# Icelk/fractal-renderer

Measured on AMD Instinct MI355X. Metric: pixel_iterations_per_sec, higher is better.
Workload: dtype f64

## Files before the change

fractal-renderer_amd/csrc/fr_api.hip:

```cpp
#include <hip/hip_runtime.h>

#include <atomic>
#include <cmath>
#include <cstddef>
#include <cstdint>
#include <cstdio>
#include <cstdlib>
#include <cstring>
#include <mutex>
#include <shared_mutex>
#include <string>
#include <vector>

#include "fr_ctx.h"

static_assert(sizeof(fr_config) == 104 && offsetof(fr_config, limit) == 16 && offsetof(fr_config, inside) == 72 &&
                  offsetof(fr_config, primary_color) == 74 && offsetof(fr_config, color_weight) == 80 &&
                  offsetof(fr_config, julia_set) == 88,
              "fr_config must stay the #[repr(C)] image of calc::Config");
static_assert(sizeof(fr_render_opts) == 32, "fr_render_opts is part of the ABI");

namespace fr {

namespace {

thread_local std::string tl_error;
thread_local Profiling tl_prof;
std::atomic<bool> g_process_exiting{false};

std::shared_mutex g_life;
std::mutex g_primary_mu;
Ctx g_primary;
bool g_primary_inited = false;

std::atomic<int> g_tile{0};
std::atomic<int> g_palette_enabled{1};
std::atomic<int> g_cycle_shortcut{0};
std::atomic<int> g_refill_minrun{-1}, g_refill_quit16{-1};
std::atomic<int> g_loop_mode{-1};
std::atomic<int> g_colour_filter{1};
std::atomic<unsigned long long *> g_queue_trace{nullptr};
std::atomic<uint32_t> g_two_pass_list_entries{0};

bool valid_tile(int tile) {
    switch (tile) {
    case 0: case 1: case 2: case 4: case 8: case 9: case 10: case 11: case 12: case 13: case 14: case 15: case 16: case 6401: case 3202: case 1604: case 808:
        return true;
    default:
        return false;
    }
}

}

int fail(int code, const char *what) {
    tl_error = what;
    return code;
}
int fail(int code, const std::string &what) {
    tl_error = what;
    return code;
}

int fail_hip(hipError_t e, const char *what) {
    char buf[512];
    snprintf(buf, sizeof buf, "%s: %s (%s)", what, hipGetErrorString(e), hipGetErrorName(e));
    tl_error = buf;
    (void)hipGetLastError();
    return (e == hipErrorNoDevice || e == hipErrorInvalidDevice) ? FR_ERR_NO_DEVICE : FR_ERR_HIP;
}

const std::string &last_error() { return tl_error; }

LifeShared::LifeShared() { g_life.lock_shared(); }
LifeShared::~LifeShared() { g_life.unlock_shared(); }
LifeExclusive::LifeExclusive() { g_life.lock(); }
LifeExclusive::~LifeExclusive() { g_life.unlock(); }

Profiling &profiling() { return tl_prof; }
Profiling::~Profiling() {
    if (e0 && !g_process_exiting.load()) {
        (void)hipEventDestroy(e0);
        (void)hipEventDestroy(e1);
    }
    e0 = e1 = nullptr;
}

Opts default_opts() {
    Opts o;
    o.tile = g_tile.load();
    o.loop_mode = g_loop_mode.load();
    o.palette = g_palette_enabled.load();
    o.cycle_shortcut = g_cycle_shortcut.load();
    o.refill_minrun = g_refill_minrun.load();
    o.refill_quit16 = g_refill_quit16.load();
    o.colour_filter = g_colour_filter.load();
    return o;
}

int resolve_opts(const fr_render_opts *in, Opts &o) {
    o = default_opts();
    if (!in) return FR_OK;
    if (in->size < sizeof(fr_render_opts)) return fail(FR_ERR_INVALID_ARGUMENT, "fr_render_opts.size is too small (use fr_render_opts_init)");
    if (!valid_tile(in->tile)) return fail(FR_ERR_INVALID_ARGUMENT, "opts.tile must be 0, 1, 2, 4, 8, 9, 10 ... 16, 6401, 3202, 1604 or 808");
    if (in->loop_mode != -1 && in->loop_mode != 0 && in->loop_mode != 2 && in->loop_mode != 4 && in->loop_mode != 5)
        return fail(FR_ERR_INVALID_ARGUMENT, "opts.loop_mode must be -1 (auto), 0, 2, 4 or 5");
    if (in->refill_minrun < -1 || in->refill_quit16 < -1 || in->refill_quit16 == 0 || in->refill_quit16 > 16)
        return fail(FR_ERR_INVALID_ARGUMENT, "opts: refill_minrun >= 0, 1 <= refill_quit16 <= 16 (or -1: the kernel's default)");
    o.tile = in->tile;
    o.loop_mode = in->loop_mode;
    o.palette = in->palette != 0;
    o.cycle_shortcut = in->cycle_shortcut != 0;
    o.refill_minrun = in->refill_minrun;
    o.refill_quit16 = in->refill_quit16;
    o.colour_filter = in->colour_filter == 2 ? 2 : in->colour_filter != 0;
    return FR_OK;
}


int Ctx::create(int device) {
    HIP_TRY(hipSetDevice(device));
    hip_device = device;
    HIP_TRY(hipStreamCreateWithFlags(&stream, hipStreamNonBlocking));
    HIP_TRY(hipStreamCreateWithFlags(&stream2, hipStreamNonBlocking));
    int prio_least = 0, prio_greatest = 0;
    if (hipDeviceGetStreamPriorityRange(&prio_least, &prio_greatest) != hipSuccess) {
        (void)hipGetLastError();
        prio_greatest = 0;
    }
    HIP_TRY(hipStreamCreateWithPriority(&copy_stream, hipStreamNonBlocking, prio_greatest));
    HIP_TRY(hipStreamCreateWithPriority(&aux_stream, hipStreamNonBlocking, prio_greatest));
    HIP_TRY(hipStreamCreateWithPriority(&aux2_stream, hipStreamNonBlocking, prio_least));
    HIP_TRY(hipMalloc(reinterpret_cast<void **>(&sample_counters), 16 * sizeof(unsigned long long)));
    HIP_TRY(hipMemset(sample_counters, 0, 16 * sizeof(unsigned long long)));
    HIP_TRY(hipHostMalloc(reinterpret_cast<void **>(&sample_result), (kViewChoices + 1) * 8 * sizeof(unsigned long long), hipHostMallocMapped));
    memset(sample_result, 0, (kViewChoices + 1) * 8 * sizeof(unsigned long long));
    for (ViewChoice &v : view_choices) HIP_TRY(hipEventCreateWithFlags(&v.after, hipEventDisableTiming));
    constexpr size_t kSlotWords = FR_MAX_PALETTE_ENTRIES + FR_SURV_QUEUES * FR_SURV_COUNT_STRIDE;
    HIP_TRY(hipMalloc(reinterpret_cast<void **>(&palette_block), sizeof(uint32_t) * kSlotWords * kPaletteSlots));
    for (int k = 0; k < kPaletteSlots; k++) {
        palette_slots[k].dev = palette_block + (size_t)k * kSlotWords;
        HIP_TRY(hipEventCreateWithFlags(&palette_slots[k].done, hipEventDisableTiming));
// ... 319 lines not shown
    p.pos_re = cfg->pos.re;
    p.pos_im = cfg->pos.im;
    p.scale_re = cfg->scale.re;
    p.scale_im = cfg->scale.im;
    p.exposure = cfg->exposure;
    p.julia_re = cfg->julia_set.re;
    p.julia_im = cfg->julia_set.im;
    p.inside = cfg->inside ? 1u : 0u;
    p.smooth = cfg->smooth ? 1u : 0u;
    p.prim[0] = cfg->primary_color.r;
    p.prim[1] = cfg->primary_color.g;
    p.prim[2] = cfg->primary_color.b;
    p.sec[0] = cfg->secondary_color.r;
    p.sec[1] = cfg->secondary_color.g;
    p.sec[2] = cfg->secondary_color.b;
    for (int k = 0; k < 3; k++) {
        p.prim_f[k] = (double)p.prim[k];
        p.sec_f[k] = (double)p.sec[k];
    }
    p.iterations_f64 = (double)cfg->iterations;
    const uint32_t n = cfg->iterations;
    p.inv_iterations = (n != 0 && (n & (n - 1)) == 0) ? 1.0 / (double)n : 0.0;
    p.ncols = cfg->width;
    p.nrows = 0;
    p.x_first = 0;
    p.x_stride = 1;
    p.block_rows = 1;
    p.y_first = 0;
    p.y_stride = 1;
    p.refill_minrun = o.refill_minrun < 0 ? 32u : (uint32_t)o.refill_minrun;
    p.refill_quit16 = o.refill_quit16 < 0 ? 8u : (uint32_t)o.refill_quit16;
    p.queue_minrun = (o.refill_minrun < 0 || (o.tile >= 11 && o.tile <= 16)) ? 8u : (uint32_t)o.refill_minrun;
    p.first_keep = ((o.tile >= 11 && o.tile <= 16) && o.refill_quit16 > 0) ? 4u * (uint32_t)o.refill_quit16 : 0u;
    p.two_pass_cap = ((o.tile >= 11 && o.tile <= 16) && o.refill_minrun > 0) ? (uint32_t)o.refill_minrun : 0u;
    p.queue_want = (o.refill_quit16 < 0 || (o.tile >= 11 && o.tile <= 16)) ? 24u : (64u * (uint32_t)o.refill_quit16 + 15u) / 16u;
    {
        static const int dbg_want = getenv("FR_DEBUG_QUEUE_WANT") ? atoi(getenv("FR_DEBUG_QUEUE_WANT")) : 0;
        static const int dbg_minrun = getenv("FR_DEBUG_QUEUE_MINRUN") ? atoi(getenv("FR_DEBUG_QUEUE_MINRUN")) : -1;
        if (dbg_want > 0 && dbg_want <= 64) p.queue_want = (uint32_t)dbg_want;
        if (dbg_minrun >= 0) p.queue_minrun = (uint32_t)dbg_minrun;
    }
    {
        static const int dbg_ablate = getenv("FR_DEBUG_ABLATE") ? atoi(getenv("FR_DEBUG_ABLATE")) : 0;
        p.debug_ablate = (uint32_t)dbg_ablate & 3u;
    }
    p.cycle_shortcut = (o.cycle_shortcut && cfg->iterations < (1u << 30)) ? 1u : 0u;
    p.filt_k = n != 0 ? cfg->exposure / (double)n : 0.0;
    const bool filter_ok = o.colour_filter && cfg->smooth && n != 0 && std::isfinite(cfg->exposure) &&
                           std::fabs(p.filt_k) <= 1e100 && cfg->stable_limit >= 0.0;
    p.colour_filter = filter_ok ? 1u : 0u;
    const double ak = std::fabs(p.filt_k);
    p.colour_filter32 = (filter_ok && o.colour_filter == 1 && n < (1u << 24) && ak >= 0x1p-60 && ak <= 0x1p60) ? 1u : 0u;
    p.filt_k32 = (float)p.filt_k;
    p.filt_c32 = p.colour_filter32 ? std::nextafterf((float)(ak * FR_NU_BRACKET * (1.0 + 0x1p-9)), INFINITY) : 0.0f;
    for (int k = 0; k < 3; k++) {
        p.filt_d[k] = p.prim_f[k] * ak * FR_NU_BRACKET * (1.0 + 0x1p-20);
        p.filt_d32[k] = p.colour_filter32 ? std::nextafterf((float)(p.prim_f[k] * ak * FR_NU_BRACKET * (1.0 + 0x1p-10)), INFINITY) : 0.0f;
        p.prim32[k] = (float)p.prim[k];
    }
    const double lo = std::fmax(cfg->stable_limit, 2.0) * (1.0 + 0x1p-20);
    p.filt_lo32 = (p.colour_filter32 && lo < 1e30) ? std::nextafterf((float)lo, INFINITY) : INFINITY;
}

static double host_coord(double coord, double max, double offset, double pos, double scale) {
    return ((coord / max) - offset) / scale + pos;
}

constexpr uint32_t kSpecQuiet = 16;

void plan_loop(const fr_config *cfg, int precision, const Opts &o, fr_kparams &p) {
    p.loop_mode = 0;
    p.skip_t = 0.0;
    p.loop_spec = 0;
    const bool no_spec = o.loop_mode == 5;
    const int forced = no_spec ? -1 : o.loop_mode;
    if (cfg->algo != FR_ALGO_MANDELBROT && cfg->algo != FR_ALGO_JULIA) return;
    if (p.ncols == 0 || p.nrows == 0) return;
    const bool f32 = precision == FR_PRECISION_F32;
    const double range_hi = f32 ? 0x1p30 : 0x1p400;
    const double slack = f32 ? 1.0 + 0x1p-18 : 1.0 + 0x1p-30;
    double lim2;
    if (f32) {
        const float lf = (float)cfg->limit;
        lim2 = (double)(lf * lf);
    } else {
        lim2 = cfg->limit * cfg->limit;
    }
    auto mag = [f32](double v) { return std::fabs(f32 ? (double)(float)v : v); };
    const double w = (double)cfg->width, h = (double)cfg->height;
    const uint64_t x_last = (uint64_t)p.x_first + (uint64_t)(p.ncols - 1) * p.x_stride;
    const uint32_t r_last = p.nrows - 1;
    const uint64_t y_last = (uint64_t)p.y_first + (uint64_t)(r_last / p.block_rows) * p.y_stride + r_last % p.block_rows;
    if (x_last > 0xFFFFFFFFull || y_last > 0xFFFFFFFFull) return;
    auto nmax = [](double a, double b) { return (a != a || b != b) ? NAN : std::fmax(a, b); };
    double smax = 0.0;
    for (double x : {(double)p.x_first, (double)x_last})
        smax = nmax(smax, mag(host_coord(x, h, (w / h) / 2.0, cfg->pos.re, cfg->scale.re)));
    for (double y : {(double)p.y_first, (double)y_last})
        smax = nmax(smax, mag(host_coord(y, h, 0.5, cfg->pos.im, cfg->scale.im)));
    const double cmax = cfg->algo == FR_ALGO_JULIA ? nmax(mag(cfg->julia_set.re), mag(cfg->julia_set.im)) : smax;
    if (!no_spec && lim2 >= 16.0 && lim2 <= (f32 ? 0x1p100 : 0x1p1000) && cmax <= lim2 / 8.0 && smax <= (f32 ? 0x1p120 : 0x1p1000)) {
        static const int dbg = getenv("FR_DEBUG_SPEC_QUIET") ? atoi(getenv("FR_DEBUG_SPEC_QUIET")) : 0;
        p.loop_spec = dbg > 0 ? (uint32_t)dbg : kSpecQuiet;
    }
    if (forced == 0) return;
    if (!(std::fabs(cfg->limit) <= range_hi)) return;
    if (!(cmax <= range_hi)) return;
    for (int m : {4, 2}) {
        if (forced > 0 && forced != m) continue;
        double d = lim2;
        for (int j = 1; j < m && d > 0.0; j++) d = std::sqrt(d / (2.0 * slack)) - cmax;
        double t = d * (1.0 - 0x1p-20);
        if (f32) {
            float tf = (float)t;
            if ((double)tf > t) tf = std::nextafterf(tf, 0.0f);
            t = (double)tf;
        }
        if (t >= 4.5 || (forced == m && t > 0.0)) {
            p.loop_mode = (uint32_t)m;
            p.skip_t = t;
            if (!(t < lim2)) p.loop_spec = 0;
            return;
        }
    }
}

static int check_rows(const fr_config *cfg, uint32_t y0, uint32_t y1) {
    if (!cfg) return fail(FR_ERR_INVALID_ARGUMENT, "cfg is NULL");
    if (y0 > y1) return fail(FR_ERR_INVALID_ARGUMENT, "y0 > y1");
    if (y1 > cfg->height) return fail(FR_ERR_INVALID_ARGUMENT, "y1 > height");
    return FR_OK;
}

int check_precision(int precision) {
    if (precision == FR_PRECISION_DD)
        return fail(FR_ERR_INVALID_ARGUMENT, "FR_PRECISION_DD is single-device only: the row renders, fr_pixel_p, fr_escape_rows(_dd) "
                                             "and fr_count_iterations take it");
    if (precision == FR_PRECISION_PT)
        return fail(FR_ERR_INVALID_ARGUMENT, "FR_PRECISION_PT is single-device only: the row renders, fr_pixel_p, fr_escape_rows(_pt) "
                                             "and fr_count_iterations take it");
    if (precision != FR_PRECISION_F64 && precision != FR_PRECISION_F32)
        return fail(FR_ERR_INVALID_ARGUMENT, "precision must be FR_PRECISION_F64 or FR_PRECISION_F32");
    return FR_OK;
}

static int check_deep(const fr_config *cfg, const fr_imaginary *pos_lo, const char *name) {
    if (!cfg) return fail(FR_ERR_INVALID_ARGUMENT, "cfg is NULL");
    const std::string n(name);
    const double lo_re = pos_lo ? pos_lo->re : 0.0, lo_im = pos_lo ? pos_lo->im : 0.0;
    const double fields[] = {cfg->limit,    cfg->stable_limit, cfg->pos.re,       cfg->pos.im,       cfg->scale.re, cfg->scale.im,
                             cfg->exposure, cfg->color_weight, cfg->julia_set.re, cfg->julia_set.im, lo_re,         lo_im};
    for (double v : fields)
        if (!std::isfinite(v)) return fail(FR_ERR_INVALID_ARGUMENT, n + ": every field of the view must be finite");
    if (!(cfg->limit > 0.0 && cfg->limit <= 0x1p500))
// ... 446 lines not shown
    snprintf(buf, buf_len, "%s", prop.gcnArchName);
    return FR_OK;
}

void fr_config_new(fr_config *cfg, uint32_t algo) {
    if (!cfg) return;
    const bool fern = algo == FR_ALGO_BARNSLEY_FERN;
    memset(cfg, 0, sizeof *cfg);
    cfg->algo = algo;
    cfg->width = 2000;
    cfg->height = 1000;
    cfg->iterations = fern ? 10000000u : 50u;
    cfg->limit = 65536.0;
    cfg->stable_limit = 2.0;
    cfg->scale.re = 0.4;
    cfg->scale.im = 0.4;
    cfg->exposure = 2.0;
    cfg->inside = 1;
    cfg->smooth = 1;
    if (fern) {
        cfg->primary_color = fr_rgb{4, 3, 100};
        cfg->secondary_color = fr_rgb{240, 240, 240};
    } else {
        cfg->primary_color = fr_rgb{40, 255, 40};
        cfg->secondary_color = fr_rgb{240, 0, 170};
    }
    cfg->color_weight = 0.01;
}

void fr_render_opts_init(fr_render_opts *opts) {
    if (!opts) return;
    const Opts o = default_opts();
    opts->size = sizeof(fr_render_opts);
    opts->tile = o.tile;
    opts->loop_mode = o.loop_mode;
    opts->palette = o.palette;
    opts->cycle_shortcut = o.cycle_shortcut;
    opts->refill_minrun = o.refill_minrun;
    opts->refill_quit16 = o.refill_quit16;
    opts->colour_filter = o.colour_filter;
}


static int render_rows_device(const fr_config *cfg, int precision, uint32_t y0, uint32_t y1, void *d_out,
                              size_t out_len, void *hip_stream, unsigned bytes_per_pixel, const fr_render_opts *opts,
                              const fr_imaginary *pos_lo = nullptr) {
    int rc = check_rows(cfg, y0, y1);
    if (rc == FR_OK) rc = check_precision_lo(cfg, precision, pos_lo);
    Opts o;
    if (rc == FR_OK) rc = resolve_opts(opts, o);
    if (rc != FR_OK) return rc;
    const size_t need = (size_t)bytes_per_pixel * cfg->width * (size_t)(y1 - y0);
    if (need == 0) return FR_OK;
    if (!d_out) return fail(FR_ERR_INVALID_ARGUMENT, "d_out is NULL");
    if (out_len < need) return fail(FR_ERR_BUFFER_TOO_SMALL, "out_len < bytes_per_pixel*width*(y1-y0)");
    if (bytes_per_pixel == 4 && (reinterpret_cast<uintptr_t>(d_out) & 3u))
        return fail(FR_ERR_INVALID_ARGUMENT, "RGBA8 output must be 4-byte aligned");
    LifeShared ls;
    Ctx *ctx;
    rc = primary(&ctx);
    if (rc != FR_OK) return rc;
    if (precision == FR_PRECISION_DD || precision == FR_PRECISION_PT)
        return render_deep_device(*ctx, precision, cfg, pos_lo, o, y0, y1, bytes_per_pixel, d_out,
                                  static_cast<hipStream_t>(hip_stream));
    fr_kparams p;
    fill_params(cfg, o, p);
    p.nrows = y1 - y0;
// ... 371 lines not shown

int fr_set_profiling(int enabled) {
    Profiling &pr = profiling();
    pr.enabled = enabled != 0;
    if (!enabled) {
        pr.have = false;
        if (pr.e0) {
            (void)hipEventDestroy(pr.e0);
            (void)hipEventDestroy(pr.e1);
            pr.e0 = pr.e1 = nullptr;
        }
    }
    return FR_OK;
}

int fr_last_kernel_ms(float *ms) {
    if (!ms) return fail(FR_ERR_INVALID_ARGUMENT, "ms is NULL");
    Profiling &pr = profiling();
    if (!pr.have) return fail(FR_ERR_INVALID_ARGUMENT, "no profiled kernel on this thread");
    HIP_TRY(hipEventSynchronize(pr.e1));
    HIP_TRY(hipEventElapsedTime(ms, pr.e0, pr.e1));
    return FR_OK;
}

int fr_last_kernel_name(char *buf, size_t buf_len) {
    if (!buf || buf_len == 0) return fail(FR_ERR_INVALID_ARGUMENT, "buf is NULL or empty");
    Profiling &pr = profiling();
    if (!pr.have) return fail(FR_ERR_INVALID_ARGUMENT, "no profiled kernel on this thread");
    snprintf(buf, buf_len, "%s", pr.kernel);
    return FR_OK;
}

int fr_set_tile(int tile) {
    if (!valid_tile(tile)) return fail(FR_ERR_INVALID_ARGUMENT, "tile must be 0, 1, 2, 4, 8, 9, 10 ... 16, 6401, 3202, 1604 or 808");
    g_tile.store(tile);
    return FR_OK;
}

int fr_set_refill_policy(int minrun, int quit16) {
    if (minrun < -1 || quit16 < -1 || quit16 == 0 || quit16 > 16)
        return fail(FR_ERR_INVALID_ARGUMENT, "minrun >= 0, 1 <= quit16 <= 16 (or -1: the kernel's default)");
    g_refill_minrun.store(minrun);
    g_refill_quit16.store(quit16);
    return FR_OK;
}

int fr_set_cycle_shortcut(int enabled) {
    g_cycle_shortcut.store(enabled ? 1 : 0);
    return FR_OK;
}

int fr_set_palette(int enabled) {
    g_palette_enabled.store(enabled ? 1 : 0);
    return FR_OK;
}

int fr_set_colour_filter(int enabled) {
    g_colour_filter.store(enabled == 2 ? 2 : enabled ? 1 : 0);
    return FR_OK;
}

int fr_set_loop_mode(int mode) {
    if (mode != -1 && mode != 0 && mode != 2 && mode != 4 && mode != 5)
        return fail(FR_ERR_INVALID_ARGUMENT, "loop mode must be -1 (auto), 0, 2, 4 or 5");
    g_loop_mode.store(mode);
    return FR_OK;
}
// ... 123 lines not shown
```

fractal-renderer_amd/csrc/fr_ctx.h:

```cpp
#ifndef FR_CTX_H
#define FR_CTX_H

#include <hip/hip_runtime.h>

#include <atomic>
#include <cstddef>
#include <cstdint>
#include <memory>
#include <condition_variable>
#include <mutex>
#include <string>
#include <thread>
#include <vector>

#include "../../include/fractal_hip.h"
#include "fr_kernels.h"

namespace fr {

int fail(int code, const char *what);
int fail(int code, const std::string &what);
int fail_hip(hipError_t e, const char *what);
const std::string &last_error();

#define HIP_TRY(expr)                                          \
    do {                                                       \
        hipError_t e_ = (expr);                                \
        if (e_ != hipSuccess) return ::fr::fail_hip(e_, #expr); \
    } while (0)

struct Opts {
    int tile = 0;
    int loop_mode = -1;
    int palette = 1;
    int cycle_shortcut = 0;
    int refill_minrun = -1, refill_quit16 = -1;
    int colour_filter = 1;
    int kernel_hint = -2;
    bool one_band = false;
    bool no_spec = false;
    uint32_t strip_tiles = 0;
    int pending_sample = -1;
};
Opts default_opts();
int resolve_opts(const fr_render_opts *o, Opts &out);

struct Scratch {
    void *ptr = nullptr;
    size_t cap = 0;
};

struct PaletteSlot {
    uint32_t *dev = nullptr;
    hipEvent_t done = nullptr;
    bool pending = false;
    bool busy = false;
};
constexpr int kPaletteSlots = 16;

struct SurvSlot {
    void *dev = nullptr;
    hipEvent_t done = nullptr;
    bool pending = false, busy = false;
};
constexpr int kSurvSlots = 3;
// ... 147 lines not shown
```

fractal-renderer_amd/csrc/fr_kernels.h:

```cpp
#ifndef FR_KERNELS_H
#define FR_KERNELS_H

#include <hip/hip_runtime.h>
#include <stdint.h>

struct fr_kparams {
    uint32_t algo;
    uint32_t width, height;
    uint32_t iterations;
    double limit, stable_limit;
    double pos_re, pos_im, scale_re, scale_im;
    double exposure;
    double julia_re, julia_im;
    uint32_t inside, smooth;
    uint32_t prim[3], sec[3];
    double prim_f[3], sec_f[3];
    double iterations_f64, inv_iterations;
    uint32_t ncols, nrows;
    uint32_t x_first, x_stride;
    uint32_t block_rows, y_first, y_stride;
    uint32_t out_in_place;
    uint32_t out_rgba;
    uint32_t loop_mode;
    double skip_t;
    uint32_t loop_spec;
    uint32_t first_no_spec;
    const uint32_t *palette;
    uint32_t palette_entries;
    uint32_t refill_minrun, refill_quit16;
    uint32_t queue_minrun, queue_want;
    uint32_t cycle_shortcut;
    uint32_t colour_filter;
    uint32_t *work_counter;
    double filt_k;
    double filt_d[3];
    uint32_t colour_filter32;
    float filt_k32;
    float filt_c32;
    float filt_d32[3];
    float prim32[3];
    float filt_lo32;
    uint32_t first_cap;
    uint32_t first_keep;
    uint32_t two_pass_cap;
    uint32_t first_only;
    uint32_t second_v1;
    uint32_t first_one_band;
    uint32_t strip_tiles;
    uint32_t debug_ablate;
    uint32_t surv_sub_capacity;
    void *surv_z;
    uint32_t *surv_pos;
    uint32_t *surv_cnt;
    void *surv_c;
    uint32_t *surv_counts;
};

constexpr uint32_t FR_SURV_QUEUES = 64;
constexpr uint32_t FR_SURV_COUNT_STRIDE = 32;
constexpr uint32_t FR_SURV_CHUNK = 64;

constexpr double FR_NU_BRACKET = 0x1p-18;

enum fr_out_mode {
    FR_OUT_RGB = 0,
    FR_OUT_ESCAPE = 1,
    FR_OUT_COUNT = 2
};

constexpr uint32_t FR_COUNT_SLOTS = 512;

struct fr_kout {
    uint8_t *rgb;
    double *z;
    uint32_t *iters;
    unsigned long long *count;
    unsigned long long *trace;
};

hipError_t fr_launch_escape(const fr_kparams &p, int precision, int mode, const fr_kout &out, int tile,
                            hipStream_t stream, const char **kernel_name);

hipError_t fr_launch_escape_dd(const fr_kparams &p, double pos_lo_re, double pos_lo_im, int mode, const fr_kout &out,
                               bool with_lo, hipStream_t stream, const char **kernel_name);

bool fr_wants_work_queue(const fr_kparams &p, int tile);

bool fr_wants_two_pass(fr_kparams &p, int precision, int tile, int hint = -1);
// ... 31 lines not shown
```

fractal-renderer_amd/csrc/fr_kernels.hip:

```cpp
#include "fr_kernels.h"

#include <cmath>

#include <cstdlib>

#include "fr_math.h"

namespace {

#include "fr_colour.h"

constexpr int kWaves = 4;


#define FR_ORBIT_STEP(SFX, TAG)                    \
    "v_add_" SFX " %[t], %[r2], -%[i2]\n"          \
    "v_add_" SFX " %[x], %[re], %[re]\n"           \
    "v_add_" SFX " %[re], %[t], %[cre]\n"          \
    "v_mul_" SFX " %[x], %[x], %[im]\n"            \
    "v_add_" SFX " %[im], %[x], %[cim]\n"          \
    "v_mul_" SFX " %[r2], %[re], %[re]\n"          \
    "v_mul_" SFX " %[i2], %[im], %[im]\n"          \
    "v_add_" SFX " %[t], %[r2], %[i2]\n"           \
    "s_mov_b64 %[sprev], exec\n"                   \
// ... 559 lines not shown
        const bool ok = valid && d32 >= f.lo && d32 <= 0x1.ffffep119f && decided;
        packed = ok ? pk : 0u;
        todo &= ~ballot64(ok);
    }
    if (todo != 0ull) {
        bool inside_done = false;
        if (lane_in(todo)) {
            double dist;
            if constexpr (sizeof(T) == 8) {
                dist = (double)(r2 + i2);
            } else {
                const double zre = (double)re, zim = (double)im;
                dist = zre * zre + zim * zim;
            }
            FR_COLD_PARAMS(kp);
            inside_done = !(dist > kp->stable_limit);
            if (inside_done && kp->inside)
                packed = sat_u8_dev(kp->sec_f[0] * dist) | (sat_u8_dev(kp->sec_f[2] * dist) << 8) | (sat_u8_dev(kp->sec_f[1] * dist) << 16);
        }
        todo &= ~ballot64(inside_done);
    }
    if (todo != 0ull) {
        if (lane_in(todo)) {
            FR_COLD_PARAMS(kp);
            const ColourConsts cc = make_colour_consts(*kp);
            uint8_t rgb[3];
            colour_pixel<T>(cc, re, im, r2, i2, iters, lds_tab, palette, rgb);
            packed = (uint32_t)rgb[0] | ((uint32_t)rgb[1] << 8) | ((uint32_t)rgb[2] << 16);
        }
    }
    return packed;
}

template <typename T, int MODE>
__device__ __forceinline__ void render_pixel(const fr_kparams &p, const fr_kout &out, const double *s_tab,
                                             const uint32_t *s_pal, double sre, double sim, bool valid,
                                             uint32_t cx, uint32_t r, uint32_t lane, uint32_t r_out,
                                             int strip_scalable = -1, const TileOut *to = nullptr) {
    double zre = 0.0, zim = 0.0;
    T tre = 0, tim = 0, tr2 = 0, ti2 = 0;
    uint32_t iters = 0;
    const bool escape_algo = p.algo == 0  || p.algo == 2 ;
    if (valid && escape_algo) {
        const double cre = p.algo == 0 ? sre : p.julia_re;
        const double cim = p.algo == 0 ? sim : p.julia_im;
        if constexpr (sizeof(T) == 8) {
            tre = sre;
            tim = sim;
            iters = orbit_auto<double>(p.loop_mode, p.iterations, tre, tim, cre, cim, p.limit * p.limit, p.skip_t,
                                       tr2, ti2, strip_scalable, p.loop_spec);
            zre = tre;
            zim = tim;
        } else {
            tre = (float)sre, tim = (float)sim;
            const float lim = (float)p.limit;
            iters = orbit_auto<float>(p.loop_mode, p.iterations, tre, tim, (float)cre, (float)cim, lim * lim,
                                      (float)p.skip_t, tr2, ti2, strip_scalable, p.loop_spec);
            zre = (double)tre;
            zim = (double)tim;
        }
    }

    if constexpr (MODE == FR_OUT_RGB) {
        if (to != nullptr) {
            uint32_t packed = 0;
            if (escape_algo) packed = colour_packed<T>(valid, to->fast_colour, tre, tim, tr2, ti2, iters, s_tab, s_pal);
            if (valid) {
                if (to->narrow) {
                    store_packed(to->base, to->lane_off, packed, to->bpp);
                } else {
                    const uint8_t rgb[3] = {(uint8_t)packed, (uint8_t)(packed >> 8), (uint8_t)(packed >> 16)};
                    store_pixel(p, out.rgb, r_out, cx, rgb);
                }
            }
        } else if (valid) {
            uint8_t rgb[3] = {0, 0, 0};
            if (escape_algo) {
                const ColourConsts cc = make_colour_consts(p);
                colour_pixel<T>(cc, tre, tim, tr2, ti2, iters, s_tab, s_pal, rgb);
            }
            store_pixel(p, out.rgb, r_out, cx, rgb);
        }
    } else if constexpr (MODE == FR_OUT_ESCAPE) {
        if (valid) {
            const uint64_t k = (uint64_t)r * p.ncols + cx;
            if (out.z) {
                out.z[2 * k] = zre;
                out.z[2 * k + 1] = zim;
            }
            if (out.iters) out.iters[k] = iters;
        }
    } else {
        unsigned long long n = 0;
        if (valid && escape_algo) n = iters < p.iterations ? (unsigned long long)iters + 1ull : p.iterations;
        for (int off = 32; off > 0; off >>= 1) n += __shfl_down(n, off, 64);
        if (lane == 0 && n) atomicAdd(out.count + ((blockIdx.x + 131u * blockIdx.y) % FR_COUNT_SLOTS), n);
    }
}

template <typename T, int TW, int TH, int WX, int WY, int MODE>
__global__ __launch_bounds__(64 * kWaves) void escape_kernel(const fr_kparams p, const fr_kout out) {
    static_assert(TW * TH == 64 && WX * WY == kWaves, "one lane per pixel, 4 waves per workgroup");
    constexpr int BW = TW * WX, BH = TH * WY;
    __shared__ double s_tab[FR_LOG2_N * 3];
    __shared__ double s_re[BW];
    __shared__ double s_im[BH];

    const uint32_t tid = threadIdx.x;
    const uint32_t tiles_x = (p.ncols + BW - 1) / BW;
    const uint32_t bx = blockIdx.x % tiles_x, by = blockIdx.x / tiles_x;
    const uint32_t col0 = bx * BW, row0 = by * BH;

    if (MODE == FR_OUT_RGB) {
        const double *gt = &g_log2_tab[0][0];
        for (uint32_t k = tid; k < FR_LOG2_N * 3; k += 64 * kWaves) s_tab[k] = gt[k];
    }
    if (tid < BW + BH) {
        const double width = (double)p.width, height = (double)p.height;
        if (tid < BW) {
            const uint32_t x = p.x_first + (col0 + tid) * p.x_stride;
            s_re[tid] = coord_to_space((double)x, height, (width / height) / 2.0, p.pos_re, p.scale_re);
        } else {
            const uint32_t r = row0 + (tid - BW);
            const uint32_t y = p.y_first + (r / p.block_rows) * p.y_stride + r % p.block_rows;
            s_im[tid - BW] = coord_to_space((double)y, height, 0.5, p.pos_im, p.scale_im);
        }
    }
    __syncthreads();

    const uint32_t wave = tid >> 6, lane = tid & 63;
// ... 2 lines not shown
    const uint32_t cx = col0 + lx, r = row0 + ly;
    const bool valid = cx < p.ncols && r < p.nrows;
    render_pixel<T, MODE>(p, out, s_tab, nullptr, s_re[lx], s_im[ly], valid, cx, r, lane, r);
}

template <typename T>
__device__ __forceinline__ bool coords_admissible(bool julia, double julia_re, double julia_im, double coord, bool relevant) {
    constexpr T lo = ScalableRange<T>::lo, hi = ScalableRange<T>::hi;
    const T v = (T)coord;
    const T av = __builtin_fabs(v);
    const bool in_range = av >= lo && av <= hi;
    bool lane_ok;
    if (julia) {
        const T jr = __builtin_fabs((T)julia_re), ji = __builtin_fabs((T)julia_im);
        lane_ok = (v == (T)0 || in_range) && jr >= lo && jr <= hi && ji >= lo && ji <= hi;
    } else {
        lane_ok = in_range;
    }
    return __ballot(relevant && !lane_ok) == 0ull;
}
template <typename T>
__device__ __forceinline__ bool coords_admissible(const fr_kparams &p, double coord, bool relevant) {
    return coords_admissible<T>(p.algo == 2, p.julia_re, p.julia_im, coord, relevant);
}

template <typename T>
__device__ __forceinline__ bool strip_is_scalable(const fr_kparams &p, double coord_lane, uint32_t tile0, uint32_t row0,
                                                  uint32_t lane) {
    const bool relevant = lane >= 56 ? (row0 + (lane - 56) < p.nrows) : (tile0 * 8u + lane < p.ncols);
    return coords_admissible<T>(p, coord_lane, relevant);
}


template <typename T, int MODE, int kStripTiles>
__global__ __launch_bounds__(64) void escape_strip_kernel(const fr_kparams p, const fr_kout out) {
    __shared__ double s_tab[(FR_LOG2_N * 3 * 8 > FR_MAX_PALETTE_ENTRIES * 4 ? FR_LOG2_N * 3 * 8 : FR_MAX_PALETTE_ENTRIES * 4) / 8];
    const uint32_t tid = threadIdx.x;
    const uint32_t *s_pal = nullptr;
    if (MODE == FR_OUT_RGB) {
        if (p.palette != nullptr) {
            uint32_t *dst = reinterpret_cast<uint32_t *>(s_tab);
            for (uint32_t k = tid; k < p.palette_entries; k += 64) dst[k] = p.palette[k];
            s_pal = dst;
        } else if (p.smooth) {
            const double *gt = &g_log2_tab[0][0];
            for (uint32_t k = tid; k < FR_LOG2_N * 3; k += 64) s_tab[k] = gt[k];
        }
        __syncthreads();
    }
    const uint32_t lane = tid;
    const uint32_t row0 = (blockIdx.y + gridDim.y * blockIdx.z) * 8u;
    if (row0 >= p.nrows) return;
    const uint32_t lx = lane & 7u, ly = lane >> 3;
    const uint32_t r = row0 + ly;
    const double width = (double)p.width, height = (double)p.height;

    static_assert(kStripTiles <= 7, "lanes 56-63 are the row lanes");
    const bool row_lane = lane >= 56;
    const uint32_t tile0 = blockIdx.x * kStripTiles;
    uint32_t coord_u;
    if (row_lane) {
        const uint32_t rr = row0 + (lane - 56);
        coord_u = p.y_first + (rr / p.block_rows) * p.y_stride + rr % p.block_rows;
    } else {
        coord_u = p.x_first + (tile0 * 8u + lane) * p.x_stride;
    }
    const double coord_lane = coord_to_space((double)coord_u, height, row_lane ? 0.5 : (width / height) / 2.0,
                                             row_lane ? p.pos_im : p.pos_re, row_lane ? p.scale_im : p.scale_re);
    const double sim = __shfl(coord_lane, 56 + ly, 64);
    uint32_t out_row0 = row0;
    if (p.out_in_place) out_row0 = p.y_first + (row0 / p.block_rows) * p.y_stride + row0 % p.block_rows;
    const uint32_t r_out = out_row0 + ly;
    const int strip_scalable = (p.loop_mode != 0 && strip_is_scalable<T>(p, coord_lane, tile0, row0, lane)) ? 1 : 0;
    TileOut to;
    to.bpp = p.out_rgba ? 4u : 3u;
    to.narrow = (uint64_t)p.ncols * to.bpp * 8u <= 0xFFFFFFFFull;
    to.lane_off = ly * (p.ncols * to.bpp) + lx * to.bpp;
    to.fast_colour = p.colour_filter32 && p.smooth && p.palette == nullptr;
    uint8_t *const strip_base = MODE == FR_OUT_RGB ? out.rgb + ((uint64_t)out_row0 * p.ncols + (uint64_t)tile0 * 8u) * to.bpp : nullptr;

    for (int k = 0; k < kStripTiles; k++) {
        const uint32_t col0 = (tile0 + k) * 8u;
        if (col0 >= p.ncols) break;
        const double sre = __shfl(coord_lane, k * 8 + lx, 64);
        const uint32_t cx = col0 + lx;
        const bool valid = cx < p.ncols && r < p.nrows;
        to.base = strip_base + (size_t)((uint32_t)k * 8u * to.bpp);
        render_pixel<T, MODE>(p, out, s_tab, s_pal, sre, sim, valid, cx, r, lane, r_out, strip_scalable, MODE == FR_OUT_RGB ? &to : nullptr);
    }
}

__device__ __forceinline__ uint32_t wave_max_u32(uint32_t v) {
    for (int off = 32; off > 0; off >>= 1) {
        const uint32_t o = __shfl_xor(v, off, 64);
        v = o > v ? o : v;
    }
    return v;
}

template <typename T>
struct Pair;
template <>
struct Pair<float> {
    typedef float2 type;
};
template <>
struct Pair<double> {
    typedef double2 type;
};

template <typename T>
__device__ __forceinline__ bool coord_is_scalable(bool julia, double coord) {
    constexpr T lo = ScalableRange<T>::lo, hi = ScalableRange<T>::hi;
    const T v = (T)coord;
    const T av = __builtin_fabs(v);
    const bool in_range = av >= lo && av <= hi;
    return julia ? (v == (T)0 || in_range) : in_range;
}

template <typename T, int M, int kStripTiles, int kBands>
__global__ __launch_bounds__(64) void escape_first_v1_kernel(const fr_kparams p, const fr_kout out) {
// ... 493 lines not shown
#define FR_TILE_OPERANDS                                                                                         \
    : [X] "=&v"(X), [Y] "=&v"(Y), [A] "=&v"(A), [B] "=&v"(B), [t] "=&v"(t), [cnt] "=&v"(cnt), [q] "=&v"(q),      \
      [sorig] "=&s"(sorig), [srun] "=&s"(srun), [k] "+s"(k), [st] "=&s"(st), [fa] "=&s"(fa), [fb] "=&s"(fb),     \
      [fk] "=&s"(fk)                                                                                             \
    : [sre] "v"(sre), [Y0] "v"(Y0), [B0] "v"(B0), [c2re] "v"(c2re), [c2im] "v"(c2im), [t4lim] "s"(t4lim),        \
      [lim4] "s"(lim4), [kargs] "s"(kargs), [offa] "i"(offsetof(fr_kparams, prim32)),                            \
      [offb] "i"(offsetof(fr_kparams, prim32) + 8),                                                              \
      [offk] "i"(offsetof(fr_kparams, filt_k32))                                                                 \
    : "vcc", "scc", "memory"
    if constexpr (sizeof(T) == 8) {
        if constexpr (M == 4)
            asm volatile(FR_TILE_ASM("f64", "v_mov_b64", FR_SC_IT("f64") FR_SC_IT("f64") FR_SC_IT("f64"), "4.0") FR_TILE_OPERANDS);
        else
            asm volatile(FR_TILE_ASM("f64", "v_mov_b64", FR_SC_IT("f64"), "2.0") FR_TILE_OPERANDS);
    } else {
        if constexpr (M == 4)
            asm volatile(FR_TILE_ASM("f32", "v_mov_b32", FR_SC_IT("f32") FR_SC_IT("f32") FR_SC_IT("f32"), "4.0") FR_TILE_OPERANDS);
        else
            asm volatile(FR_TILE_ASM("f32", "v_mov_b32", FR_SC_IT("f32"), "2.0") FR_TILE_OPERANDS);
    }
    return st;
}

template <typename T>
__device__ __forceinline__ typename UBits<T>::type bpermute_t(uint32_t byte_index, T v) {
    if constexpr (sizeof(T) == 8) {
        const uint64_t b = fr_bits_of(v);
        const uint32_t lo = (uint32_t)__builtin_amdgcn_ds_bpermute((int)byte_index, (int)(uint32_t)b);
        const uint32_t hi = (uint32_t)__builtin_amdgcn_ds_bpermute((int)byte_index, (int)(uint32_t)(b >> 32));
        return (uint64_t)lo | ((uint64_t)hi << 32);
    } else {
        return (uint32_t)__builtin_amdgcn_ds_bpermute((int)byte_index, __builtin_bit_cast(int, v));
    }
}

template <typename T, int M, int kStripTiles, int kBands, bool SPEC = false>
__global__ __launch_bounds__(64) void escape_first_kernel(const fr_kparams p, const fr_kout out) {
    __shared__ uint32_t s_palette[FR_MAX_PALETTE_ENTRIES];
    const double *const s_tab = &g_log2_tab[0][0];
    typedef typename Pair<T>::type T2;
    typedef typename UBits<T>::type UB;
    static_assert(kStripTiles <= 8 && kBands <= 8, "one column / one row coordinate per lane");
    const uint32_t lane = threadIdx.x;
    const uint32_t lx = lane & 7u, ly = lane >> 3;
    const uint32_t *s_pal = nullptr;
    uint32_t row0, tile0, ncols, nrows, bpp, lane_pitch;
    T colsT, rowsT;
    bool cols_scalable;
    unsigned long long bad_rows;
    bool narrow;
    bool fast_colour;
    {
        FR_COLD_PARAMS(kp);
        const auto &P = *kp;
        if (P.palette != nullptr) {
            const uint32_t n = P.palette_entries;
            const uint32_t *src = P.palette;
            for (uint32_t k = lane; k < n; k += 64) s_palette[k] = src[k];
            s_pal = s_palette;
            __syncthreads();
        }
        row0 = (blockIdx.y + gridDim.y * blockIdx.z) * (8u * kBands);
        nrows = P.nrows, ncols = P.ncols;
        if (row0 >= nrows) return;
        const double width = (double)P.width, height = (double)P.height;
        tile0 = blockIdx.x * kStripTiles;
// ... 1825 lines not shown
```

Baseline: 5105 billion.

## Add straight-line fast-block path to strip kernel with fused colour filter

Splits render_pixel into orbit and output stages and adds a fast path in the strip kernel. For scalable tiles in loop mode 4, it runs a fixed number of unrolled iteration blocks through tile_fast and writes colour directly when the whole wave escapes early enough for the float32 colour filter to decide. Otherwise it resumes the orbit from the saved state. It also drops the shared-memory copy of the log2 table in favour of the global table, simplifies row coordinate maths when one block covers all rows, and adds a tile-option family (20-28) that disables the fast path. The extra control flow could add register pressure or divergence.

```diff
diff --git a/fractal-renderer_amd/csrc/fr_api.hip b/fractal-renderer_amd/csrc/fr_api.hip
--- a/fractal-renderer_amd/csrc/fr_api.hip
+++ b/fractal-renderer_amd/csrc/fr_api.hip
@@ -45,6 +45,7 @@
 bool valid_tile(int tile) {
     switch (tile) {
     case 0: case 1: case 2: case 4: case 8: case 9: case 10: case 11: case 12: case 13: case 14: case 15: case 16: case 6401: case 3202: case 1604: case 808:
+    case 20: case 21: case 22: case 24: case 28:
         return true;
     default:
         return false;
@@ -86,9 +87,14 @@
     e0 = e1 = nullptr;
 }
 
+static void set_tile(Opts &o, int tile) {
+    o.strip_general = tile >= 20 && tile <= 28;
+    o.tile = o.strip_general ? tile - 20 : tile;
+}
+
 Opts default_opts() {
     Opts o;
-    o.tile = g_tile.load();
+    set_tile(o, g_tile.load());
     o.loop_mode = g_loop_mode.load();
     o.palette = g_palette_enabled.load();
     o.cycle_shortcut = g_cycle_shortcut.load();
@@ -102,12 +108,12 @@
     o = default_opts();
     if (!in) return FR_OK;
     if (in->size < sizeof(fr_render_opts)) return fail(FR_ERR_INVALID_ARGUMENT, "fr_render_opts.size is too small (use fr_render_opts_init)");
-    if (!valid_tile(in->tile)) return fail(FR_ERR_INVALID_ARGUMENT, "opts.tile must be 0, 1, 2, 4, 8, 9, 10 ... 16, 6401, 3202, 1604 or 808");
+    if (!valid_tile(in->tile)) return fail(FR_ERR_INVALID_ARGUMENT, "opts.tile must be 0, 1, 2, 4, 8, 9, 10 ... 16, 20, 21, 22, 24, 28, 6401, 3202, 1604 or 808");
     if (in->loop_mode != -1 && in->loop_mode != 0 && in->loop_mode != 2 && in->loop_mode != 4 && in->loop_mode != 5)
         return fail(FR_ERR_INVALID_ARGUMENT, "opts.loop_mode must be -1 (auto), 0, 2, 4 or 5");
     if (in->refill_minrun < -1 || in->refill_quit16 < -1 || in->refill_quit16 == 0 || in->refill_quit16 > 16)
         return fail(FR_ERR_INVALID_ARGUMENT, "opts: refill_minrun >= 0, 1 <= refill_quit16 <= 16 (or -1: the kernel's default)");
-    o.tile = in->tile;
+    set_tile(o, in->tile);
     o.loop_mode = in->loop_mode;
     o.palette = in->palette != 0;
     o.cycle_shortcut = in->cycle_shortcut != 0;
@@ -493,6 +499,7 @@
     p.refill_quit16 = o.refill_quit16 < 0 ? 8u : (uint32_t)o.refill_quit16;
     p.queue_minrun = (o.refill_minrun < 0 || (o.tile >= 11 && o.tile <= 16)) ? 8u : (uint32_t)o.refill_minrun;
     p.first_keep = ((o.tile >= 11 && o.tile <= 16) && o.refill_quit16 > 0) ? 4u * (uint32_t)o.refill_quit16 : 0u;
+    p.strip_general_only = o.strip_general ? 1u : 0u;
     p.two_pass_cap = ((o.tile >= 11 && o.tile <= 16) && o.refill_minrun > 0) ? (uint32_t)o.refill_minrun : 0u;
     p.queue_want = (o.refill_quit16 < 0 || (o.tile >= 11 && o.tile <= 16)) ? 24u : (64u * (uint32_t)o.refill_quit16 + 15u) / 16u;
     {
@@ -528,11 +535,28 @@
 }
 
 constexpr uint32_t kSpecQuiet = 16;
+constexpr uint32_t kStripEpisode = 16;
+static uint32_t strip_episode() {
+    static const int dbg = getenv("FR_DEBUG_STRIP_EPISODE") ? atoi(getenv("FR_DEBUG_STRIP_EPISODE")) : 0;
+    return (dbg >= 4 && dbg <= 64) ? ((uint32_t)dbg & ~3u) : kStripEpisode;
+}
+static uint64_t bits_of_f64(double v) {
+    uint64_t b;
+    memcpy(&b, &v, sizeof b);
+    return b;
+}
+static uint64_t bits_of_f32(float v) {
+    uint32_t b;
+    memcpy(&b, &v, sizeof b);
+    return b;
+}
 
 void plan_loop(const fr_config *cfg, int precision, const Opts &o, fr_kparams &p) {
     p.loop_mode = 0;
     p.skip_t = 0.0;
     p.loop_spec = 0;
+    p.strip_fast_blocks = 0;
+    p.lim4_bits = p.t4_bits = 0;
     const bool no_spec = o.loop_mode == 5;
     const int forced = no_spec ? -1 : o.loop_mode;
     if (cfg->algo != FR_ALGO_MANDELBROT && cfg->algo != FR_ALGO_JULIA) return;
@@ -581,6 +605,16 @@
             p.loop_mode = (uint32_t)m;
             p.skip_t = t;
             if (!(t < lim2)) p.loop_spec = 0;
+            if (f32) {
+                const float lf = (float)cfg->limit;
+                p.lim4_bits = bits_of_f32(4.0f * (lf * lf));
+                p.t4_bits = bits_of_f32(4.0f * (float)t);
+            } else {
+                p.lim4_bits = bits_of_f64(4.0 * (cfg->limit * cfg->limit));
+                p.t4_bits = bits_of_f64(4.0 * t);
+            }
+            if (m == 4 && !p.strip_general_only && cfg->iterations < (1u << 24) && strip_episode() + 64u <= cfg->iterations)
+                p.strip_fast_blocks = strip_episode() / 4u;
             return;
         }
     }
@@ -1093,7 +1127,7 @@
     if (!opts) return;
     const Opts o = default_opts();
     opts->size = sizeof(fr_render_opts);
-    opts->tile = o.tile;
+    opts->tile = o.strip_general ? o.tile + 20 : o.tile;
     opts->loop_mode = o.loop_mode;
     opts->palette = o.palette;
     opts->cycle_shortcut = o.cycle_shortcut;
@@ -1531,7 +1565,7 @@
 }
 
 int fr_set_tile(int tile) {
-    if (!valid_tile(tile)) return fail(FR_ERR_INVALID_ARGUMENT, "tile must be 0, 1, 2, 4, 8, 9, 10 ... 16, 6401, 3202, 1604 or 808");
+    if (!valid_tile(tile)) return fail(FR_ERR_INVALID_ARGUMENT, "tile must be 0, 1, 2, 4, 8, 9, 10 ... 16, 20, 21, 22, 24, 28, 6401, 3202, 1604 or 808");
     g_tile.store(tile);
     return FR_OK;
 }
diff --git a/fractal-renderer_amd/csrc/fr_ctx.h b/fractal-renderer_amd/csrc/fr_ctx.h
--- a/fractal-renderer_amd/csrc/fr_ctx.h
+++ b/fractal-renderer_amd/csrc/fr_ctx.h
@@ -31,6 +31,7 @@
 
 struct Opts {
     int tile = 0;
+    bool strip_general = false;
     int loop_mode = -1;
     int palette = 1;
     int cycle_shortcut = 0;
diff --git a/fractal-renderer_amd/csrc/fr_kernels.h b/fractal-renderer_amd/csrc/fr_kernels.h
--- a/fractal-renderer_amd/csrc/fr_kernels.h
+++ b/fractal-renderer_amd/csrc/fr_kernels.h
@@ -54,6 +54,9 @@
     uint32_t *surv_cnt;
     void *surv_c;
     uint32_t *surv_counts;
+    uint32_t strip_fast_blocks;
+    uint32_t strip_general_only;
+    uint64_t lim4_bits, t4_bits;
 };
 
 constexpr uint32_t FR_SURV_QUEUES = 64;
diff --git a/fractal-renderer_amd/csrc/fr_kernels.hip b/fractal-renderer_amd/csrc/fr_kernels.hip
--- a/fractal-renderer_amd/csrc/fr_kernels.hip
+++ b/fractal-renderer_amd/csrc/fr_kernels.hip
@@ -615,14 +615,10 @@
     return packed;
 }
 
-template <typename T, int MODE>
-__device__ __forceinline__ void render_pixel(const fr_kparams &p, const fr_kout &out, const double *s_tab,
-                                             const uint32_t *s_pal, double sre, double sim, bool valid,
-                                             uint32_t cx, uint32_t r, uint32_t lane, uint32_t r_out,
-                                             int strip_scalable = -1, const TileOut *to = nullptr) {
-    double zre = 0.0, zim = 0.0;
-    T tre = 0, tim = 0, tr2 = 0, ti2 = 0;
-    uint32_t iters = 0;
+template <typename T>
+__device__ __forceinline__ void orbit_pixel(const fr_kparams &p, double sre, double sim, bool valid, int strip_scalable, T &tre,
+                                            T &tim, T &tr2, T &ti2, uint32_t &iters) {
+    tre = 0, tim = 0, tr2 = 0, ti2 = 0, iters = 0;
     const bool escape_algo = p.algo == 0  || p.algo == 2 ;
     if (valid && escape_algo) {
         const double cre = p.algo == 0 ? sre : p.julia_re;
@@ -632,18 +628,20 @@
             tim = sim;
             iters = orbit_auto<double>(p.loop_mode, p.iterations, tre, tim, cre, cim, p.limit * p.limit, p.skip_t,
                                        tr2, ti2, strip_scalable, p.loop_spec);
-            zre = tre;
-            zim = tim;
         } else {
             tre = (float)sre, tim = (float)sim;
             const float lim = (float)p.limit;
             iters = orbit_auto<float>(p.loop_mode, p.iterations, tre, tim, (float)cre, (float)cim, lim * lim,
                                       (float)p.skip_t, tr2, ti2, strip_scalable, p.loop_spec);
-            zre = (double)tre;
-            zim = (double)tim;
-        }
-    }
-
+        }
+    }
+}
+
+template <typename T, int MODE>
+__device__ __forceinline__ void output_pixel(const fr_kparams &p, const fr_kout &out, const double *s_tab, const uint32_t *s_pal,
+                                             bool valid, uint32_t cx, uint32_t r, uint32_t lane, uint32_t r_out, T tre, T tim,
+                                             T tr2, T ti2, uint32_t iters, const TileOut *to = nullptr) {
+    const bool escape_algo = p.algo == 0 || p.algo == 2;
     if constexpr (MODE == FR_OUT_RGB) {
         if (to != nullptr) {
             uint32_t packed = 0;
@@ -668,8 +666,8 @@
         if (valid) {
             const uint64_t k = (uint64_t)r * p.ncols + cx;
             if (out.z) {
-                out.z[2 * k] = zre;
-                out.z[2 * k + 1] = zim;
+                out.z[2 * k] = (double)tre;
+                out.z[2 * k + 1] = (double)tim;
             }
             if (out.iters) out.iters[k] = iters;
         }
@@ -679,6 +677,17 @@
         for (int off = 32; off > 0; off >>= 1) n += __shfl_down(n, off, 64);
         if (lane == 0 && n) atomicAdd(out.count + ((blockIdx.x + 131u * blockIdx.y) % FR_COUNT_SLOTS), n);
     }
+}
+
+template <typename T, int MODE>
+__device__ __forceinline__ void render_pixel(const fr_kparams &p, const fr_kout &out, const double *s_tab,
+                                             const uint32_t *s_pal, double sre, double sim, bool valid,
+                                             uint32_t cx, uint32_t r, uint32_t lane, uint32_t r_out,
+                                             int strip_scalable = -1, const TileOut *to = nullptr) {
+    T tre, tim, tr2, ti2;
+    uint32_t iters;
+    orbit_pixel<T>(p, sre, sim, valid, strip_scalable, tre, tim, tr2, ti2, iters);
+    output_pixel<T, MODE>(p, out, s_tab, s_pal, valid, cx, r, lane, r_out, tre, tim, tr2, ti2, iters, to);
 }
 
 template <typename T, int TW, int TH, int WX, int WY, int MODE>
@@ -747,21 +756,65 @@
 }
 
 
+template <typename T>
+__device__ __forceinline__ int strip_tile_straight(const fr_kparams &p, uint32_t nblk, T sre, T Y0, T B0, T c2re, T c2im,
+                                                   const TileOut &to, T &X, T &Y, T &A, T &B, unsigned long long &run, uint32_t &iters);
+
+template <typename T>
+__device__ __forceinline__ void strip_orbit(const fr_kparams &p, double sre, double sim, bool valid, int strip_scalable, bool resume,
+                                            unsigned long long run, uint32_t done, T X, T Y, T A, T B, T &tre, T &tim, T &tr2, T &ti2,
+                                            uint32_t &iters) {
+    const bool escape_algo = p.algo == 0  || p.algo == 2 ;
+    const bool julia = p.algo == 2;
+    const T cre = julia ? (T)p.julia_re : (T)sre;
+    const T cim = julia ? (T)p.julia_im : (T)sim;
+    T squared, skip_t;
+    if constexpr (sizeof(T) == 8) {
+        squared = p.limit * p.limit, skip_t = p.skip_t;
+    } else {
+        const float lim = (float)p.limit;
+        squared = lim * lim, skip_t = (float)p.skip_t;
+    }
+    if (p.loop_mode == 4 && strip_scalable == 1) {
+        bool go = lane_in(run);
+        uint32_t n = p.iterations - done;
+        if (!resume) {
+            X = (T)sre + (T)sre, Y = (T)sim + (T)sim, A = X * X, B = Y * Y;
+            go = valid && escape_algo;
+            n = p.iterations, done = 0, iters = 0;
+        }
+        if (go) {
+            uint32_t completed;
+            const uint32_t it = orbit_scaled_run<T, 4, false>(n, X, Y, A, B, cre + cre, cim + cim, squared, skip_t, EpisodeCtl{0, 0},
+                                                              completed, nullptr, nullptr, nullptr, p.loop_spec);
+            iters = done + it;
+        }
+        tre = X * (T)0.5, tim = Y * (T)0.5;
+        tr2 = tre * tre, ti2 = tim * tim;
+    } else {
+        tre = 0, tim = 0, tr2 = 0, ti2 = 0, iters = 0;
+        if (valid && escape_algo) {
+            tre = (T)sre, tim = (T)sim;
+            if (p.loop_mode != 0 && strip_scalable == 1)
+                iters = orbit_scaled<T, 2>(p.iterations, tre, tim, cre, cim, squared, skip_t, tr2, ti2);
+            else
+                iters = orbit<T>(p.iterations, tre, tim, cre, cim, squared, tr2, ti2, p.loop_spec);
+        }
+    }
+}
+
 template <typename T, int MODE, int kStripTiles>
 __global__ __launch_bounds__(64) void escape_strip_kernel(const fr_kparams p, const fr_kout out) {
-    __shared__ double s_tab[(FR_LOG2_N * 3 * 8 > FR_MAX_PALETTE_ENTRIES * 4 ? FR_LOG2_N * 3 * 8 : FR_MAX_PALETTE_ENTRIES * 4) / 8];
+    __shared__ uint32_t s_palette[FR_MAX_PALETTE_ENTRIES];
+    const double *const s_tab = &g_log2_tab[0][0];
     const uint32_t tid = threadIdx.x;
     const uint32_t *s_pal = nullptr;
     if (MODE == FR_OUT_RGB) {
         if (p.palette != nullptr) {
-            uint32_t *dst = reinterpret_cast<uint32_t *>(s_tab);
-            for (uint32_t k = tid; k < p.palette_entries; k += 64) dst[k] = p.palette[k];
-            s_pal = dst;
-        } else if (p.smooth) {
-            const double *gt = &g_log2_tab[0][0];
-            for (uint32_t k = tid; k < FR_LOG2_N * 3; k += 64) s_tab[k] = gt[k];
-        }
-        __syncthreads();
+            for (uint32_t k = tid; k < p.palette_entries; k += 64) s_palette[k] = p.palette[k];
+            s_pal = s_palette;
+            __syncthreads();
+        }
     }
     const uint32_t lane = tid;
     const uint32_t row0 = (blockIdx.y + gridDim.y * blockIdx.z) * 8u;
@@ -774,34 +827,59 @@
     const bool row_lane = lane >= 56;
     const uint32_t tile0 = blockIdx.x * kStripTiles;
     uint32_t coord_u;
+    const bool one_block = p.block_rows >= p.nrows;
     if (row_lane) {
         const uint32_t rr = row0 + (lane - 56);
-        coord_u = p.y_first + (rr / p.block_rows) * p.y_stride + rr % p.block_rows;
+        coord_u = one_block ? p.y_first + rr : p.y_first + (rr / p.block_rows) * p.y_stride + rr % p.block_rows;
     } else {
         coord_u = p.x_first + (tile0 * 8u + lane) * p.x_stride;
     }
     const double coord_lane = coord_to_space((double)coord_u, height, row_lane ? 0.5 : (width / height) / 2.0,
                                              row_lane ? p.pos_im : p.pos_re, row_lane ? p.scale_im : p.scale_re);
-    const double sim = __shfl(coord_lane, 56 + ly, 64);
+    double sim = __shfl(coord_lane, 56 + ly, 64);
     uint32_t out_row0 = row0;
-    if (p.out_in_place) out_row0 = p.y_first + (row0 / p.block_rows) * p.y_stride + row0 % p.block_rows;
+    if (p.out_in_place) out_row0 = one_block ? p.y_first + row0 : p.y_first + (row0 / p.block_rows) * p.y_stride + row0 % p.block_rows;
     const uint32_t r_out = out_row0 + ly;
     const int strip_scalable = (p.loop_mode != 0 && strip_is_scalable<T>(p, coord_lane, tile0, row0, lane)) ? 1 : 0;
     TileOut to;
     to.bpp = p.out_rgba ? 4u : 3u;
     to.narrow = (uint64_t)p.ncols * to.bpp * 8u <= 0xFFFFFFFFull;
     to.lane_off = ly * (p.ncols * to.bpp) + lx * to.bpp;
-    to.fast_colour = p.colour_filter32 && p.smooth && p.palette == nullptr;
+    to.fast_colour = MODE == FR_OUT_RGB && p.colour_filter32 && p.smooth && p.palette == nullptr;
     uint8_t *const strip_base = MODE == FR_OUT_RGB ? out.rgb + ((uint64_t)out_row0 * p.ncols + (uint64_t)tile0 * 8u) * to.bpp : nullptr;
+
+    uint32_t fast_blocks = 0;
+    if (p.strip_fast_blocks != 0u && strip_scalable == 1 && row0 + 8u <= p.nrows && to.narrow) fast_blocks = p.strip_fast_blocks;
 
     for (int k = 0; k < kStripTiles; k++) {
         const uint32_t col0 = (tile0 + k) * 8u;
         if (col0 >= p.ncols) break;
         const double sre = __shfl(coord_lane, k * 8 + lx, 64);
+        asm volatile("" : "+v"(sim));
         const uint32_t cx = col0 + lx;
         const bool valid = cx < p.ncols && r < p.nrows;
         to.base = strip_base + (size_t)((uint32_t)k * 8u * to.bpp);
-        render_pixel<T, MODE>(p, out, s_tab, s_pal, sre, sim, valid, cx, r, lane, r_out, strip_scalable, MODE == FR_OUT_RGB ? &to : nullptr);
+        T X = 0, Y = 0, A = 0, B = 0;
+        unsigned long long run = 0ull;
+        uint32_t iters = 0, done = 0;
+        bool resume = false;
+        {
+            if (fast_blocks != 0u && col0 + 8u <= p.ncols) {
+                const T sre_t = (T)sre;
+                const T sim_t = (T)sim;
+                const T Y0 = sim_t + sim_t, B0 = Y0 * Y0;
+                const bool julia = p.algo == 2;
+                const T c2re = julia ? (T)p.julia_re + (T)p.julia_re : sre_t + sre_t;
+                const T c2im = julia ? (T)p.julia_im + (T)p.julia_im : Y0;
+                const int how = strip_tile_straight<T>(p, fast_blocks, sre_t, Y0, B0, c2re, c2im, to, X, Y, A, B, run, iters);
+                if (how == 0) continue;
+                resume = how == 1;
+                done = fast_blocks * 4u;
+            }
+        }
+        T tre, tim, tr2, ti2;
+        strip_orbit<T>(p, sre, sim, valid, strip_scalable, resume, run, done, X, Y, A, B, tre, tim, tr2, ti2, iters);
+        output_pixel<T, MODE>(p, out, s_tab, s_pal, valid, cx, r, lane, r_out, tre, tim, tr2, ti2, iters, MODE == FR_OUT_RGB ? &to : nullptr);
     }
 }
 
@@ -1361,6 +1439,70 @@
     } else {
         return (uint32_t)__builtin_amdgcn_ds_bpermute((int)byte_index, __builtin_bit_cast(int, v));
     }
+}
+
+template <typename T>
+__device__ __forceinline__ int strip_tile_straight(const fr_kparams &p, uint32_t nblk, T sre, T Y0, T B0, T c2re, T c2im,
+                                                   const TileOut &to, T &X, T &Y, T &A, T &B, unsigned long long &run, uint32_t &iters) {
+    typedef typename UBits<T>::type UB;
+    const UB t4lim = (UB)p.t4_bits, lim4 = (UB)p.lim4_bits;
+    T t;
+    float cnt;
+    unsigned long long fa, fb, fk;
+    run = 0ull;
+    const uint32_t st = tile_fast<T, 4>(__builtin_amdgcn_readfirstlane(nblk), sre, Y0, B0, c2re, c2im, t4lim, lim4,
+                                        (KArgs)__builtin_amdgcn_kernarg_segment_ptr(), X, Y, A, B, t, cnt, run, fa, fb, fk);
+    if (st == 2u) return 2;
+    if (st == 0u) {
+        if (to.fast_colour) {
+            Filter32 fc;
+            fc.lo = __builtin_bit_cast(float, (uint32_t)(fb >> 32));
+            fc.k = __builtin_bit_cast(float, (uint32_t)fk), fc.c = __builtin_bit_cast(float, (uint32_t)(fk >> 32));
+            fc.p0 = __builtin_bit_cast(float, (uint32_t)fa), fc.p1 = __builtin_bit_cast(float, (uint32_t)fb);
+            fc.p2 = __builtin_bit_cast(float, (uint32_t)(fa >> 32));
+            const float d32 = (float)t * 0.25f;
+            const bool unsure = !(d32 >= fc.lo && d32 <= 0x1.ffffep119f);
+            if (ballot64(unsure) == 0ull) {
+                uint32_t pk;
+                const bool decided = colour_fast32(fc, d32, cnt, pk);
+                if (ballot64(!decided) == 0ull) {
+                    store_packed(to.base, to.lane_off, pk, to.bpp);
+                    return 0;
+                }
+            }
+        }
+        iters = (uint32_t)cnt - 1u;
+        run = 0ull;
+        return 1;
+    }
+    FR_COLD_PARAMS(kp);
+    const uint32_t cap = kp->iterations, k1 = nblk * 4u;
+    const T lim4v = __builtin_bit_cast(T, lim4);
+    unsigned long long esc, live;
+    uint32_t bound;
+    if (st == 1u) {
+        const unsigned long long frozen = ~run;
+        esc = ballot64(t > lim4v) & frozen;
+        live = frozen & ~esc;
+        bound = k1;
+    } else {
+        live = run, esc = ~run, run = 0ull;
+        bound = k1 + 64u;
+    }
+    while (live != 0ull) {
+        uint32_t nf = 64u;
+        if (bound + 64u > cap) {
+            live &= ~ballot64((uint32_t)cnt >= cap);
+            if (live == 0ull) break;
+            nf = 1u;
+        }
+        const unsigned long long still = finish_scaled<T>(live, nf, X, Y, A, B, t, cnt, c2re, c2im, lim4);
+        esc |= live & ~still;
+        live = still;
+        bound += nf;
+    }
+    iters = lane_in(esc) ? (uint32_t)cnt - 1u : cap;
+    return 1;
 }
 
 template <typename T, int M, int kStripTiles, int kBands, bool SPEC = false>
```

Measured after the change: 5188 billion (median of 6 runs). 1.02x the previous value.
